# luigiba/OpenKEonSpark

Hardware: AMD Instinct MI355X
Metric: positive triples/sec (training step) (higher is better)
Workload: dtype f32

## Files before the change

### openkeonspark_amd/csrc/abi.hip

```cpp
#include <cstdio>
#include <cstring>
#include <iostream>

#include "engine.hpp"

namespace kge {

Engine &engine() {
    static Engine e;
    return e;
}

void set_error(const std::string &msg) {
    engine().last_error = msg;
    std::fprintf(stderr, "[kge_mi355] error: %s\n", msg.c_str());
}

int fail(int code, const std::string &msg) {
    set_error(msg);
    return code;
}

int hip_check(hipError_t e, const char *what) {
    if (e == hipSuccess) return KGE_OK;
// ... 141 lines not shown
INT getWorkThreads(void) { return engine().work_threads; }
void setBern(INT con) { engine().bern = con; }

void randReset(void) {
    Engine &e = engine();
    e.streams.resize((size_t)e.work_threads);
    for (auto &s : e.streams) s = (uint64_t)(int64_t)e.libc.next();
    e.dev.streams_sync = 0;
}

void importTrainFiles(void) {
    Engine &e = engine();
    std::printf("The toolkit is importing datasets.\n");
    int64_t E = 0, R = 0, nb = 0;
    std::vector<int64_t> h, t, r;
    std::string err = load_openke_dir(e.in_path, E, R, nb, h, t, r);
    if (!err.empty()) {
        std::cout << err << std::endl;
        set_error(err);
        return;
    }
    std::printf("The total of relations is %ld.\n", (long)R);
    std::printf("The total of entities is %ld.\n", (long)E);
    if (nb > 0) std::printf("The total number of new batch triples is: %ld\n", (long)nb);
    std::printf("The total of train triples is %ld.\n", (long)h.size());
    err = build_and_adopt(E, R, nb, (int64_t)h.size(), h.data(), t.data(), r.data());
    if (!err.empty()) { set_error(err); return; }
    std::fflush(stdout);
}

INT getEntityTotal(void) { return engine().index.ent_total; }
INT getRelationTotal(void) { return engine().index.rel_total; }
INT kge_eval_test_total(void); INT kge_eval_valid_total(void); INT kge_eval_triple_total(void);
INT getTripleTotal(void) { return kge_eval_triple_total(); }
INT getTrainTotal(void) { return engine().index.train_uniq; }
INT getTrainTotal_(void) { return engine().index.train_dup; }
INT getBatchTotal(void) { return engine().index.new_batch; }
INT getTestTotal(void) { return kge_eval_test_total(); }
INT getValidTotal(void) { return kge_eval_valid_total(); }

void sampling(INT *batch_h, INT *batch_t, INT *batch_r, REAL *batch_y, INT batchSize, INT negRate, INT negRelRate) {
    Engine &e = engine();
    if (ensure_device_index()) return;
    if (batchSize <= 0 || negRate < 0 || negRelRate < 0) { set_error("sampling: bad sizes"); return; }
    const int64_t total = batchSize * (1 + negRate + negRelRate);
    if (e.dev.stage_i32.reserve(3 * total, "alloc stage")) return;
    if (e.dev.stage_i64.reserve((int64_t)(sizeof(int64_t) * 3 + sizeof(float)) * total, "alloc stage")) return;
    int32_t *s = e.dev.stage_i32;
    if (launch_sampler(s, s + total, s + 2 * total, batchSize, negRate, negRelRate, 0, e.work_threads, batchSize, nullptr, nullptr)) return;
    int64_t *w = reinterpret_cast<int64_t *>(e.dev.stage_i64.ptr());
    if (launch_widen(s, w, batchSize, total, nullptr)) return;
    if (hip_check(hipMemcpy(batch_h, w, sizeof(int64_t) * total, hipMemcpyDeviceToHost), "copy batch_h")) return;
    if (hip_check(hipMemcpy(batch_t, w + total, sizeof(int64_t) * total, hipMemcpyDeviceToHost), "copy batch_t")) return;
    if (hip_check(hipMemcpy(batch_r, w + 2 * total, sizeof(int64_t) * total, hipMemcpyDeviceToHost), "copy batch_r")) return;
    hip_check(hipMemcpy(batch_y, w + 3 * total, sizeof(float) * total, hipMemcpyDeviceToHost), "copy batch_y");
}

size_t kge_last_error(char *buf, size_t n) {
    const std::string &s = engine().last_error;
    if (buf && n) {
        size_t k = s.size() < n - 1 ? s.size() : n - 1;
        std::memcpy(buf, s.data(), k);
        buf[k] = 0;
    }
    return s.size();
}

void kge_clear_error(void) { engine().last_error.clear(); }
int kge_device_available(void) { return device_ok() ? 1 : 0; }
const char *kge_version(void) { return "kge_mi355 0.1 (gfx950)"; }

int kge_set_option(const char *name, INT value) {
    std::string n = name ? name : "";
    if (n == "counts_force_sort") { engine().counts_force_sort = value != 0; return KGE_OK; }
    if (n == "sampler_magic_len") {
        Engine &e = engine();
        if (device_ok()) { (void)flush_attached_sampler(nullptr); (void)hipDeviceSynchronize(); }
        e.sampler_magic_len = value > 0 ? value : 0;
        if (e.index.loaded) build_magic_tables(e.index, e.sampler_magic_len);
        e.dev.tables_uploaded = false;
        return KGE_OK;
    }
    if (n == "counts_sort_tiles") { engine().counts_sort_tiles = value > 0 ? (int)value : 0; return KGE_OK; }
    if (n == "ride_shares") { engine().ride_shares = (int)value; return KGE_OK; }
    if (n == "transr_bf16x3") { engine().transr_bf16x3 = value != 0; return KGE_OK; }
    if (n == "transr_groups") { engine().transr_groups = (int)value; return KGE_OK; }
    if (n == "transr_fuse_vec") { engine().transr_fuse_vec = value != 0; return KGE_OK; }
    if (n == "shared_transr_stages") { engine().shared_transr_stages = value >= 1 && value <= 5 ? (int)value : 5; return KGE_OK; }
    if (n == "counts_fused") { engine().counts_fused = value != 0; return KGE_OK; }
    if (n == "counts_fused_diag") { engine().counts_fused_diag = (int)value; return KGE_OK; }
    if (n == "counts_fused_cap") { engine().counts_fused_cap = value > 0 ? (int)value : 0; return KGE_OK; }
    if (n == "counts_fused_tail") { engine().counts_fused_tail = value != 0; return KGE_OK; }
    if (n == "inv_table_max_bytes") { engine().inv_table_max_bytes = value; return KGE_OK; }
    if (n == "tables_changed") { tables_written(); return KGE_OK; }
    if (n == "counts_krel") { int k = 1; while (k * 2 <= value && k < 64) k *= 2; engine().counts_krel = k; return KGE_OK; }
    if (n == "inv_carry") { engine().inv_carry = value != 0; tables_written(); return KGE_OK; }
    if (n == "emit_rounds") { engine().emit_rounds = value != 0; return KGE_OK; }
    if (n == "emit_pack") { engine().emit_pack = value != 0; return KGE_OK; }
    if (n == "emit_keys_grouped") { engine().emit_keys_grouped = value != 0; return KGE_OK; }
    if (n == "counts_sort_test_group") { engine().counts_sort_test_group = value > 0 ? (int)value : 0; return KGE_OK; }
    if (n == "float_records") { engine().float_records = value != 0; return KGE_OK; }
    if (n == "float_records_min") { engine().float_records_min = value; return KGE_OK; }
    if (n == "index_device_min") { engine().index_device_min = value; return KGE_OK; }
    if (n == "eval_index_device_min") { engine().eval_index_device_min = value; return KGE_OK; }
    if (n == "hub_copies") { engine().hub_copies = value != 0; return KGE_OK; }
    if (n == "pair_counts") { engine().pair_counts = value != 0; return KGE_OK; }
    if (n == "record_emit_event") { engine().record_emit_event = value != 0; return KGE_OK; }
    if (n == "transr_dgrad_records") { engine().transr_dgrad_records = value != 0; return KGE_OK; }
    if (n == "transr_dgrad_records_min") { engine().transr_dgrad_records_min = value; return KGE_OK; }
    if (n == "transr_lean") { engine().transr_lean = value != 0; return KGE_OK; }
    if (n == "pair_counts_min_neg") { engine().pair_counts_min_neg = (int)value; return KGE_OK; }
    if (n == "topk_table_max_bytes") { engine().topk_table_max_bytes = value; return KGE_OK; }
    if (n == "relpred_chunk_bytes") { engine().relpred_chunk_bytes = value; return KGE_OK; }
    if (n == "lp_v1") { engine().lp_v1 = value != 0; return KGE_OK; }
    if (n == "rank_slices") { engine().rank_slices = value > 0 ? (int)value : 0; return KGE_OK; }
    if (n == "rankc_slices") { engine().rankc_slices = value > 0 ? (int)value : 0; return KGE_OK; }
    if (n == "rankc_fused") { engine().rankc_fused = value != 0; return KGE_OK; }
    if (n == "transr_v1") { engine().transr_v1 = (int)value; return KGE_OK; }
    if (n == "time_emit") { engine().time_emit = value > 0 ? (int)value : 0; if (value > 0) { engine().emit_launches = 0; engine().emit_seen = 0; } return KGE_OK; }
    if (n == "time_sampler") { engine().time_sampler = value > 0 ? (int)value : 0; if (value > 0) { engine().samp_launches = 0; engine().samp_seen = 0; } return KGE_OK; }
    if (n == "fb_occ4") { engine().fb_occ4 = value != 0; return KGE_OK; }
    if (n == "persist_ahead") { engine().persist_ahead = value != 0; return KGE_OK; }
    if (n == "persist_touch") { engine().persist_touch = value != 0; return KGE_OK; }
    if (n == "persist_trace") { engine().persist_trace = value != 0; return KGE_OK; }
    if (n == "persist_threads") { engine().persist_threads = value == 1024 ? 1024 : 512; return KGE_OK; }
    if (n == "libc_rand_restart") { engine().libc = LibcRand(); return KGE_OK; }
    return fail(KGE_ERR_BAD_ARG, "kge_set_option: unknown option " + n);
}

int kge_last_kernel_ms(const char *name, float *ms) {
    Engine &e = engine();
    std::string n = name ? name : "";
    if ((n != "transe_emit" && n != "sampler") || !ms) return fail(KGE_ERR_BAD_ARG, "kge_last_kernel_ms: unknown kernel " + n);
    const bool samp = n == "sampler";
    const long long done = samp ? e.samp_launches : e.emit_launches;
    hipEvent_t *ev0 = samp ? e.ev_samp0 : e.ev_emit0, *ev1 = samp ? e.ev_samp1 : e.ev_emit1;
    if (done <= 0) return fail(KGE_ERR_BAD_ARG, "kge_last_kernel_ms: enable option time_emit / time_sampler and run a step first");
    const int slot = (int)((done - 1) % Engine::kEmitRing);
    if (hip_check(hipEventSynchronize(ev1[slot]), "event sync")) return KGE_ERR_NO_DEVICE;
    return hip_check(hipEventElapsedTime(ms, ev0[slot], ev1[slot]), "event elapsed");
}

int kge_kernel_ms_mean(const char *name, float *mean_ms, INT *launches) {
    Engine &e = engine();
    std::string n = name ? name : "";
    if ((n != "transe_emit" && n != "sampler") || !mean_ms) return fail(KGE_ERR_BAD_ARG, "kge_kernel_ms_mean: unknown kernel " + n);
    const bool samp = n == "sampler";
    const long long done = samp ? e.samp_launches : e.emit_launches;
    hipEvent_t *ev0 = samp ? e.ev_samp0 : e.ev_emit0, *ev1 = samp ? e.ev_samp1 : e.ev_emit1;
    const long long have = done < Engine::kEmitRing ? done : (long long)Engine::kEmitRing;
    if (have <= 0) return fail(KGE_ERR_BAD_ARG, "kge_kernel_ms_mean: enable option time_emit / time_sampler and run steps first");
    double sum = 0.0;
    for (long long i = 0; i < have; i++) {
        const int slot = (int)((done - 1 - i) % Engine::kEmitRing);
        float ms = 0.f;
        if (hip_check(hipEventSynchronize(ev1[slot]), "event sync")) return KGE_ERR_NO_DEVICE;
        if (hip_check(hipEventElapsedTime(&ms, ev0[slot], ev1[slot]), "event elapsed")) return KGE_ERR_NO_DEVICE;
        sum += ms;
    }
    *mean_ms = (float)(sum / (double)have);
    if (launches) *launches = have;
    return KGE_OK;
}

int kge_import_train_arrays(INT ent_total, INT rel_total, INT n, const INT *h, const INT *t, const INT *r,
                            INT new_batch_total) {
// ... 339 lines not shown
```

### openkeonspark_amd/csrc/engine.hpp

```cpp
#pragma once
#include <hip/hip_runtime.h>

#include <cstdint>
#include <mutex>
#include <string>
#include <vector>

#include "../../include/kge_mi355.h"
#include "dev_buf.hpp"
#include "kg_index.hpp"

namespace kge {

struct DeviceIndex {
    bool uploaded = false;
    DevBuf<int4> pos, grp;
    DevBuf<int2> ht;
    DevBuf<int32_t> tails_hr, heads_tr, rels_ht;
    DevBuf<float> bern_prob;
    bool tables_uploaded = false;
    DevBuf<LcgAffine> jump_digits;
    DevBuf<uint64_t> ent_magic, rel_magic;
    DevBuf<uint64_t> streams_buf;
    uint64_t *streams = nullptr;
    uint64_t *streams_next = nullptr;
    int streams_sync = 0;
    DevBuf<int32_t> stage_i32;
    DevBuf<char> stage_i64;
    DevBuf<float> loss_partials;
    DevBuf<unsigned> loss_ticket;
    bool typed_uploaded = false;
    DevBuf<int2> typed_len;
    DevBuf<int4> type_bounds;
    DevBuf<int32_t> type_tails, type_heads, typed_pos_hr, typed_pos_tr;
};

struct Engine {
    std::mutex mu;
    std::string in_path = "../data/FB15K/";
    std::string out_path = "../data/FB15K/";
    int64_t work_threads = 1;
    int64_t bern = 0;
    KgIndex index;
    unsigned long long index_generation = 0;
    LibcRand libc;
    std::vector<uint64_t> streams;
    LcgJumpTable jump = make_jump_table();
    std::vector<LcgAffine> jump_digits = make_jump_digit_table(jump);
    int64_t sampler_magic_len = 2048;
    DeviceIndex dev;
    std::string last_error;
    int device_state = 0;
    int record_emit_event = 0;
    hipEvent_t emit_done = nullptr;
    unsigned long long emit_seq = 0, emit_waited = 0;
    int time_emit = 0;
    static constexpr int kEmitRing = 512;
    hipEvent_t ev_emit0[kEmitRing] = {}, ev_emit1[kEmitRing] = {};
    long long emit_launches = 0;
    long long emit_seen = 0;
    int time_sampler = 0;
    hipEvent_t ev_samp0[kEmitRing] = {}, ev_samp1[kEmitRing] = {};
    long long samp_launches = 0, samp_seen = 0;
    DevBuf<float> inv_norm;
    const float *inv_for_ent = nullptr, *inv_for_rel = nullptr;
    int inv_valid = 0;
    int32_t *loss_limbs = nullptr;
    int counts_krel = 4;
    int inv_carry = 1;
    int emit_rounds = 1;
    int emit_pack = 1;
    int emit_keys_grouped = 1;
    int counts_sort_test_group = 0;
    int64_t inv_table_max_bytes = int64_t(256) << 20;
    int float_records = 1;
    int64_t float_records_min = 1 << 16;
    int64_t index_device_min = int64_t(1) << 22;
    int64_t eval_index_device_min = int64_t(1) << 22;
    int transr_dgrad_records = 1;
    int64_t transr_dgrad_records_min = 1 << 15;
    int transr_bf16x3 = 1;
    int transr_groups = 1;
    int transr_fuse_vec = 1;
    int shared_transr_stages = 5;
    int transr_lean = 1;
    int pair_counts = 1;
    int pair_counts_min_neg = 0;
    int hub_copies = 1;
    int64_t topk_table_max_bytes = int64_t(1) << 30;
    int64_t relpred_chunk_bytes = int64_t(256) << 20;
    int lp_v1 = 0;
    int rank_slices = 0;
    int rankc_slices = 0;
    int rankc_fused = 1;
    int transr_v1 = 0;
    int fb_occ4 = 1;
    int persist_ahead = 1;
    int persist_touch = 0;
    int persist_trace = 0;
    int persist_threads = 512;
    int counts_force_sort = 0;
    int counts_sort_tiles = 1;
    int ride_shares = -1;
    int counts_fused = 1;
    int counts_fused_diag = 0;
    int typed_sampling = 0;
    int counts_fused_cap = 0;
    int counts_fused_tail = 1;
};

Engine &engine();
inline void tables_written() { engine().inv_valid = 0; }
struct SamplerArgs;
bool take_attached_sampler(SamplerArgs &a, unsigned &blocks, float share = 1.0f);
int flush_attached_sampler(hipStream_t stream);
int attach_sampler(int32_t *d_h, int32_t *d_t, int32_t *d_r, int64_t B, int64_t neg, int64_t negrel, int64_t thread_lo,
                   int64_t thread_hi, int64_t out_stride, int64_t *n_local_out, hipStream_t stream, int32_t *d_pack = nullptr);
void set_error(const std::string &msg);
int fail(int code, const std::string &msg);
bool device_ok();
int ensure_device_index();
int ensure_typed_index(bool always = false);
int ensure_typed_host_index();
struct TypeListsHost { const std::vector<int32_t> *head_lef, *head_rig, *head_type, *tail_lef, *tail_rig, *tail_type; };
bool eval_type_lists_host(TypeListsHost &v);

constexpr int kMaxLossBlocks = 4096;

struct NegClass { bool same_h, same_t, same_r, fast; };
template <int MODEL>
__host__ __device__ inline NegClass classify_negative(long long h, long long t, long long r, long long nh,
                                                               long long nt, long long nr, int negative_rel) {
    NegClass c;
    c.same_r = nr == r;
    const bool ctx_same = MODEL == KGE_TRANSE ? true : (MODEL == KGE_TRANSR ? (negative_rel == 0 || c.same_r) : c.same_r);
    c.same_h = nh == h && ctx_same;
    c.same_t = nt == t && ctx_same;
    c.fast = ((int)!c.same_h + (int)!c.same_t + (int)!c.same_r) == 1;
    return c;
}



struct FloatRowSpace {
    float *g_ent, *g_rel, *g_auxr, *g_auxe;
    long long E, R;
    long long hub_base, hub_rows;
    long long rows;
    float scale = 1.0f;
};
bool pair_path_active(const kge_model_desc &m, int64_t n_pos, int64_t n_neg);
bool transr_group_layout_active(const kge_model_desc &m, int64_t n_pos, int64_t n_neg);
int transe_relation_copies(const kge_model_desc &m, int64_t n_pos);
int float_records_chunk_len(int64_t M);
int sgd_rows_skipped(int32_t *out);
int float_records_workspace(int64_t M, int D, float *&rec, int32_t *&dst);
int float_records_reduce(int64_t M, int D, const FloatRowSpace &rs, hipStream_t stream, const float *rec_ext = nullptr, int32_t *dst_ext = nullptr,
                         bool deterministic = false);
enum { kRuleAdam = 0, kRuleAdagrad = 1, kRuleRowAdagrad = 2 };
struct RowRule {
    float *m[4], *v[4];
    float lr_t, b1, b2, eps;
    int rule;
};
int float_records_reduce_adam(int64_t M, int D, const FloatRowSpace &rs, const RowRule &ad, hipStream_t stream, const float *rec_ext = nullptr,
                              int32_t *dst_ext = nullptr);
int launch_forward_backward_records(const kge_model_desc &m, const float *const tables[4], const int32_t *d_h, const int32_t *d_t,
                                    const int32_t *d_r, int64_t n_pos, int64_t n_neg, int64_t stride, int64_t denom, int64_t n_pos_total,
                                    float *d_rec, int32_t *d_dst, int64_t rec_offset, int64_t rec_slice, float *d_loss, hipStream_t stream);
int launch_float_records_apply_adam(const kge_model_desc &m, float *const tables[4], const RowRule &ad, const float *d_rec, int32_t *d_dst,
                                    int64_t M_total, int64_t n_pos_total, int64_t n_neg, hipStream_t stream);
int launch_float_records_apply(const kge_model_desc &m, float *const tables[4], const float *d_rec, int32_t *d_dst, int64_t M_total,
                               int64_t n_pos_total, int64_t n_neg, float lr, hipStream_t stream);
void float_record_hubs(const kge_model_desc &m, int64_t n_pos_total, int64_t n_neg, int64_t &hub_base, int64_t &hub_k, int64_t &rows);

bool device_index_build_supported(int64_t E, int64_t R, int64_t n);
std::string build_index_device(KgIndex &ix, DeviceIndex &dev, int64_t E, int64_t R, int64_t new_batch, int64_t n, const int64_t *h,
                               const int64_t *t, const int64_t *r);

int launch_sampler(int32_t *d_h, int32_t *d_t, int32_t *d_r, int64_t B, int64_t neg, int64_t negrel, int64_t thread_lo,
                   int64_t thread_hi, int64_t out_stride, int64_t *n_local, hipStream_t stream, int32_t *d_pack = nullptr);
inline int sampler_kshift(int64_t neg, int64_t negrel) { int k = 0; while ((int64_t(1) << k) < 1 + neg + negrel) k++; return k; }
constexpr int kPackRowBits = 28;
inline bool emit_pack_shape(int64_t ent_total, int64_t rel_total, int64_t neg, int64_t negrel) {
    return engine().emit_pack && sampler_kshift(neg, negrel) <= 6 && neg + negrel >= 1 && ent_total < (int64_t(1) << kPackRowBits) &&
// ... 40 lines not shown
```

### openkeonspark_amd/csrc/transe_counts.hip

```cpp
#include <cstring>
#include <string.h>

#include <rocprim/rocprim.hpp>

#include "engine.hpp"
#include "team.hpp"
#include "team_shape.hpp"
#include "sampler_dev.hpp"
#include "optim_dev.hpp"

namespace kge {

void transe_team_shape(int D, int &L, int &C);
int launch_transe_emit(const kge_model_desc &m, const float *ent, const float *rel, float *resid_ent, float *resid_rel,
                       const int32_t *d_h, const int32_t *d_t, const int32_t *d_r, int64_t n_pos, int64_t n_neg, int64_t stride,
                       int64_t denom, uint32_t *rec, int32_t *dst, int krel, float *d_loss, hipStream_t stream, bool track_deferred,
                       uint8_t *rec2 = nullptr, const int32_t *neg_pack = nullptr, bool keys_grouped = false);
bool transe_emit_groups_keys(int D);

int transe_deferred_groups(int32_t *out);

namespace {

int bits_for_rows(int64_t v) { int b = 1; while ((int64_t(1) << b) <= v) b++; return b; }
// ... 414 lines not shown
        if (threadIdx.x < 64) {
            int v[4], tot = 0;
#pragma unroll
            for (int k = 0; k < 4; k++) { v[k] = span_sum[4 * threadIdx.x + k]; tot += v[k]; }
            int incl = tot;
#pragma unroll
            for (int off = 1; off < 64; off <<= 1) { const int t = __shfl_up(incl, off); if ((int)threadIdx.x >= off) incl += t; }
            int run = incl - tot;
#pragma unroll
            for (int k = 0; k < 4; k++) { span_sum[4 * threadIdx.x + k] = run; run += v[k]; }
        }
        __syncthreads();
        int run = span_sum[threadIdx.x];
        for (int i = lo; i < hi; i++) { const int c = lds_h[i]; lds_h[i] = run; run += c; }
    }
    __syncthreads();
#pragma unroll
    for (int k = 0; k < PC; k++)
        if (start + (int)threadIdx.x + 256 * k < end) {
            const int pos = start + atomicAdd(&lds_h[pr[k].y - row0], 1);
            out_keys[pos] = pr[k].y;
            out_ids[pos] = pr[k].x;
        }
    for (int i = 256 * PC + threadIdx.x; i < n; i += 256) {
        const int2 q = fetch(i);
        const int pos = start + atomicAdd(&lds_h[q.y - row0], 1);
        out_keys[pos] = q.y;
        out_ids[pos] = q.x;
    }
    if constexpr (PLAN) {
        __syncthreads();
        const int cap = plan.cap;
        for (int i = threadIdx.x; i < rpb; i += 256) {
            const int key = row0 + i;
            if (key >= rows) break;
            const int lo = i ? lds_h[i - 1] : 0, c = lds_h[i] - lo;
            plan.row_span[key] = make_int2(start + lo, c);
            const int io = i ^ 1;
            const int co = lds_h[io] - (io ? lds_h[io - 1] : 0);
            if (c > 0 && (c > cap || co > cap)) {
                const int np = (c + cap - 1) / cap;
                const int base = atomicAdd(plan.n_pieces, np);
                for (int q = 0; q < np; q++) plan.pieces[base + q] = make_int4(key, start + lo + q * cap, min(cap, c - q * cap), 0);
            }
            if (plan.expect && !(i & 1)) plan_arrivals(plan, key >> 1, c, co);
        }
    }
}

template <bool PLAN>
__global__ __launch_bounds__(256) void bkt_sort_kernel(const int2 *__restrict__ pairs, const int32_t *__restrict__ bucket_start,
                                                       int rpb, int rows, int32_t *__restrict__ out_keys,
                                                       int32_t *__restrict__ out_ids, int32_t *__restrict__ bucket_total,
                                                       int32_t *__restrict__ cursor, SegPlan plan, SamplerArgs ride) {
    extern __shared__ int lds_h[];
    if ((int)blockIdx.x >= NB) {
        __shared__ float bern_lds[kBernLds];
        sample_block_ride(ride, (long long)blockIdx.x - NB, bern_lds);
        return;
    }
    const int b = blockIdx.x;
    const int row0 = b * rpb;
    if (threadIdx.x == 0) {
        bucket_total[b] = 0; cursor[b] = 0;
        if (b == 0) { bucket_total[NB] = 0; cursor[NB] = 0; }
    }
    if (row0 >= rows) return;
    const int start = bucket_start[b], end = bucket_start[b + 1];
    bucket_rows_sort<PLAN>(row0, start, end, rpb, rows, lds_h, out_keys, out_ids, plan, [&](int i) { return pairs[start + i]; });
}


template <bool PLAN>
static void launch_bkt_sort(int2 *pairs, int rpb, int rows, int32_t *totals, int32_t *cursor, const SegPlan &plan, hipStream_t stream) {
    SamplerArgs ride = {};
    const unsigned n_ride = take_ride(ride, 2);
    hipLaunchKernelGGL(bkt_sort_kernel<PLAN>, dim3(NB + n_ride), dim3(256), sizeof(int) * (size_t)rpb, stream, pairs, g_c.bucket_start, rpb, rows,
                       g_c.dst_sorted, g_c.ids_sorted, totals, cursor, plan, ride);
}

constexpr int kSortTile = 2048;
constexpr int kSortMaxTiles = 2048;
constexpr int kOffStride = NB + 1;

struct KeyMap {
    unsigned S, magic, shift;
    int n_pos;
};
static KeyMap key_map_for(int S, int64_t n_pos) {
    KeyMap k;
    k.S = (unsigned)S; k.n_pos = (int)n_pos;
    unsigned sh = 0;
    while ((2u << sh) <= (unsigned)S) sh++;
    if ((1u << sh) == (unsigned)S) { k.magic = 0x80000000u; k.shift = sh - 1; }
    else {
        k.magic = (unsigned)(((uint64_t(1) << (32 + sh)) + (unsigned)S - 1) / (unsigned)S); k.shift = sh;
    }
    return k;
}
__device__ __forceinline__ int key_id_of(unsigned S, unsigned magic, unsigned shift, int n_pos, int p) {
    const unsigned b = __umulhi((unsigned)p, magic) >> shift;
    return (int)(((unsigned)p - b * S) * (unsigned)n_pos + b);
}

template <int T, bool GROUPED = false>
__global__ __launch_bounds__(256) void bkt_tile_kernel(const int32_t *__restrict__ dst, int M, int rpb, int2 *__restrict__ tile_pairs,
                                                       int32_t *__restrict__ tile_off, int32_t *__restrict__ plan_counter, SamplerArgs ride,
                                                       int n_tiles, unsigned km_S, unsigned km_magic, unsigned km_shift, int km_n_pos) {
    if ((int)blockIdx.x >= n_tiles) {
        __shared__ float bern_lds[kBernLds];
        sample_block_ride(ride, (long long)blockIdx.x - n_tiles, bern_lds);
        return;
    }
    constexpr int K = T / 256;
    __shared__ int hist[NB];
    __shared__ int wave_total[4];
    __shared__ int2 stage[T];
    if (plan_counter && blockIdx.x == 0 && threadIdx.x == 0) plan_counter[0] = 0;
    const int base = blockIdx.x * T;
    int d[K], code[K];
#pragma unroll
    for (int k = 0; k < K; k++) {
        const int m = base + threadIdx.x + 256 * k;
        d[k] = m < M ? dst[m] : -1;
    }
    for (int i = threadIdx.x; i < NB; i += 256) hist[i] = 0;
    __syncthreads();
#pragma unroll
    for (int k = 0; k < K; k++) {
        const unsigned bk = (unsigned)d[k] / (unsigned)rpb;
        code[k] = bk < (unsigned)NB ? (int)(bk << 16) | atomicAdd(&hist[bk], 1) : -1;
    }
    __syncthreads();
    {
        const int v0 = hist[2 * threadIdx.x], v1 = hist[2 * threadIdx.x + 1], run = v0 + v1;
        const int lane = threadIdx.x & 63, wave = threadIdx.x >> 6;
        int incl = run;
#pragma unroll
        for (int off = 1; off < 64; off <<= 1) { const int t = __shfl_up(incl, off); if (lane >= off) incl += t; }
        if (lane == 63) wave_total[wave] = incl;
        __syncthreads();
        int excl = incl - run;
        for (int w = 0; w < wave; w++) excl += wave_total[w];
        hist[2 * threadIdx.x] = excl; hist[2 * threadIdx.x + 1] = excl + v0;
        int32_t *off = tile_off + (size_t)blockIdx.x * kOffStride;
        off[2 * threadIdx.x] = excl; off[2 * threadIdx.x + 1] = excl + v0;
        if (threadIdx.x == 255) off[NB] = excl + run;
    }
    __syncthreads();
    const int live = wave_total[0] + wave_total[1] + wave_total[2] + wave_total[3];
#pragma unroll
    for (int k = 0; k < K; k++)
        if (code[k] >= 0) {
            const int p = base + (int)threadIdx.x + 256 * k;
            stage[hist[code[k] >> 16] + (code[k] & 0xFFFF)] = make_int2(GROUPED ? key_id_of(km_S, km_magic, km_shift, km_n_pos, p) : p, d[k]);
        }
    __syncthreads();
    for (int i = threadIdx.x; i < live; i += 256) tile_pairs[base + i] = stage[i];
}

template <bool PLAN, int T>
__global__ __launch_bounds__(256) void bkt_merge_kernel(const int2 *__restrict__ tile_pairs, const int32_t *__restrict__ tile_off, int n_tiles,
                                                        int32_t *__restrict__ bucket_start, int M, int rpb, int rows,
                                                        int32_t *__restrict__ out_keys, int32_t *__restrict__ out_ids, SegPlan plan,
                                                        SamplerArgs ride) {
    extern __shared__ int lds_h[];
    if ((int)blockIdx.x >= NB) {
        __shared__ float bern_lds[kBernLds];
        sample_block_ride(ride, (long long)blockIdx.x - NB, bern_lds);
        return;
    }
    __shared__ int seg_pre[kSortMaxTiles + 1];
    __shared__ int seg_src[kSortMaxTiles];
    __shared__ int wave_len[4], wave_below[4];
    const int b = blockIdx.x;
    constexpr int PER = kSortMaxTiles / 256;
    const int per = (n_tiles + 255) / 256;
    const int t_lo = min((int)threadIdx.x * per, n_tiles), t_hi = min(t_lo + per, n_tiles);
    int a[PER], e[PER];
#pragma unroll
    for (int j = 0; j < PER; j++) {
        const int32_t *off = tile_off + (size_t)min(t_lo + j, max(n_tiles - 1, 0)) * kOffStride + b;
        const bool mine = t_lo + j < t_hi;
        a[j] = mine ? off[0] : 0;
        e[j] = mine ? off[1] : 0;
    }
    int len = 0, below = 0;
#pragma unroll
    for (int j = 0; j < PER; j++)
        if (t_lo + j < t_hi) {
            seg_src[t_lo + j] = (t_lo + j) * T + a[j];
            seg_pre[t_lo + j] = len;
            len += e[j] - a[j];
            below += a[j];
        }
    const int lane = threadIdx.x & 63, wave = threadIdx.x >> 6;
    int incl = len;
#pragma unroll
    for (int off = 1; off < 64; off <<= 1) { const int t = __shfl_up(incl, off); if (lane >= off) incl += t; }
#pragma unroll
    for (int off = 32; off > 0; off >>= 1) below += __shfl_xor(below, off);
    if (lane == 63) { wave_len[wave] = incl; wave_below[wave] = below; }
    __syncthreads();
    int excl = incl - len;
    for (int w = 0; w < wave; w++) excl += wave_len[w];
    for (int t = t_lo; t < t_hi; t++) seg_pre[t] += excl;
    const int start = wave_below[0] + wave_below[1] + wave_below[2] + wave_below[3];
    const int end = start + wave_len[0] + wave_len[1] + wave_len[2] + wave_len[3];
    if (threadIdx.x == 0) {
        seg_pre[n_tiles] = end - start;
        bucket_start[b] = start;
        if (b == NB - 1) { bucket_start[NB] = end; bucket_start[NB + 1] = M; }
    }
    __syncthreads();
    const int row0 = b * rpb;
    if (row0 >= rows) return;
    bucket_rows_sort<PLAN>(row0, start, end, rpb, rows, lds_h, out_keys, out_ids, plan, [&](int i) {
        int lo = 0, hi = n_tiles;
        while (hi - lo > 1) { const int mid = (lo + hi) >> 1; if (seg_pre[mid] <= i) lo = mid; else hi = mid; }
        return tile_pairs[seg_src[lo] + (i - seg_pre[lo])];
    });
}

template <int T>
static void launch_tile_sort(const int32_t *dst, int n_tiles, int M, int rows, int rpb, const SegPlan *plan, hipStream_t stream,
                             const KeyMap *km) {
    int2 *pairs = reinterpret_cast<int2 *>(g_c.pairs.ptr());
    SamplerArgs ride = {};
    unsigned n_ride = take_ride(ride, 1, true);
    if (n_tiles + n_ride > 0) {
        if (km)
            hipLaunchKernelGGL((bkt_tile_kernel<T, true>), dim3((unsigned)n_tiles + n_ride), dim3(256), 0, stream, dst, M, rpb, pairs,
                               g_c.tile_off.ptr(), plan ? plan->n_pieces : nullptr, ride, n_tiles, km->S, km->magic, km->shift, km->n_pos);
        else
            hipLaunchKernelGGL((bkt_tile_kernel<T, false>), dim3((unsigned)n_tiles + n_ride), dim3(256), 0, stream, dst, M, rpb, pairs,
                               g_c.tile_off.ptr(), plan ? plan->n_pieces : nullptr, ride, n_tiles, 0u, 0u, 0u, 0);
    }
    ride = SamplerArgs();
    n_ride = take_ride(ride, 2, true);
    if (plan)
        hipLaunchKernelGGL((bkt_merge_kernel<true, T>), dim3(NB + n_ride), dim3(256), sizeof(int) * (size_t)rpb, stream, pairs, g_c.tile_off.ptr(),
                           n_tiles, g_c.bucket_start.ptr(), M, rpb, rows, g_c.dst_sorted.ptr(), g_c.ids_sorted.ptr(), *plan, ride);
    else
        hipLaunchKernelGGL((bkt_merge_kernel<false, T>), dim3(NB + n_ride), dim3(256), sizeof(int) * (size_t)rpb, stream, pairs, g_c.tile_off.ptr(),
                           n_tiles, g_c.bucket_start.ptr(), M, rpb, rows, g_c.dst_sorted.ptr(), g_c.ids_sorted.ptr(), SegPlan(), ride);
}

__global__ void run_flags_kernel(const int32_t *__restrict__ keys, const int32_t *__restrict__ n_valid_p, int M, int32_t *__restrict__ flags) {
    const int n = n_valid_p[0];
    for (int i = blockIdx.x * blockDim.x + threadIdx.x; i < M; i += gridDim.x * blockDim.x)
        flags[i] = (i < n && (i == 0 || keys[i] != keys[i - 1])) ? 1 : 0;
}

__global__ void unique_rows_kernel(const int32_t *__restrict__ keys, const int32_t *__restrict__ n_valid_p, int32_t *__restrict__ uidx1,
                                   int32_t *__restrict__ rows_out, int32_t *__restrict__ n_rows_out, int32_t *__restrict__ S, int D,
                                   int32_t *__restrict__ bflag) {
    const int n = n_valid_p[0];
    for (int i = blockIdx.x * blockDim.x + threadIdx.x; i < n; i += gridDim.x * blockDim.x) {
        const int u = uidx1[i] - 1;
        uidx1[i] = u;
        if (i == 0 || keys[i] != keys[i - 1]) rows_out[u] = keys[i];
        if (i == n - 1) n_rows_out[0] = u + 1;
        if (bflag && ((i % CHUNK) == 0 || (i % CHUNK) == CHUNK - 1 || i == n - 1)) bflag[u] = 1;
    }
    if (n == 0 && blockIdx.x == 0 && threadIdx.x == 0) n_rows_out[0] = 0;
}

__global__ __launch_bounds__(256) void zero_boundary_rows_kernel(const int32_t *__restrict__ uidx, const int32_t *__restrict__ n_valid_p,
                                                                 int32_t *__restrict__ S, int D) {
    const int n = n_valid_p[0];
    const int lane = threadIdx.x & 63;
    const long long n_chunks = ((long long)n + CHUNK - 1) / CHUNK;
    for (long long c = (long long)blockIdx.x * 4 + (threadIdx.x >> 6); c < n_chunks; c += (long long)gridDim.x * 4) {
        const long long first = c * CHUNK, last = min(first + CHUNK, (long long)n) - 1;
        const int u0 = uidx[first], u1 = uidx[last];
        for (int e = lane; e < D; e += 64) {
            S[(long long)u0 * D + e] = 0;
            S[(long long)u1 * D + e] = 0;
        }
    }
}



__device__ __forceinline__ float *float_row_ptr(const FloatRowSpace &rs, long long row, int D) {
    if (row < rs.E) return rs.g_ent + row * D;
    if (row < rs.hub_base) return rs.g_auxe + (row - rs.E) * D;
    const long long q = (row - rs.hub_base) % rs.hub_rows;
    return q < rs.R ? rs.g_rel + q * D : rs.g_auxr + (q - rs.R) * D;
}

template <int L, int C>
__device__ __forceinline__ void flush_run_f32(const FloatRowSpace &rs, int D, int lane, long long row, const float (&acc)[C], bool atomic) {
    float *p = float_row_ptr(rs, row, D);
    atomic = atomic || row >= rs.hub_base;
#pragma unroll
    for (int c = 0; c < C; c++) {
        const int e = lane + L * c;
        if (e < D) {
            const float v = mul_rn(rs.scale, acc[c]);
            if (atomic) __builtin_amdgcn_global_atomic_fadd_f32((__attribute__((address_space(1))) float *)(p + e), v);
            else p[e] += v;
        }
    }
}

template <int L, int C>
__global__ __launch_bounds__(256) void segsum_f32_kernel(const float *__restrict__ rec, const int32_t *__restrict__ keys,
                                                         const int32_t *__restrict__ ids, const int32_t *__restrict__ n_valid_p,
                                                         FloatRowSpace rs, int D, int chunk_len) {
    constexpr int TEAMS = 256 / L;
    constexpr int U = C <= 4 ? 8 : 4;
    const int lane = threadIdx.x % L;
    const int n_valid = n_valid_p[0];
    const long long chunk = (long long)blockIdx.x * TEAMS + threadIdx.x / L;
    const long long start = chunk * chunk_len;
    if (start >= n_valid) return;
    const int n = (int)min((long long)chunk_len, n_valid - start);
    float acc[C];
#pragma unroll
    for (int c = 0; c < C; c++) acc[c] = 0.f;
    int cur = keys[start];
    bool first_run = true;
    constexpr int J = CHUNK / L;
    int kl[J], idl[J];
#pragma unroll
    for (int j = 0; j < J; j++) {
// ... 364 lines not shown
        q.row = row; q.rel = rel;
        if (row != req_row) {
            req_x = *reinterpret_cast<const float4 *>(pr.ent + (long long)row * D + lane4);
            if constexpr (MODEL == KGE_TRANSD) req_xa = *reinterpret_cast<const float4 *>(pr.auxe + (long long)row * D + lane4);
            req_row = row;
        }
        q.x = req_x;
        if constexpr (MODEL == KGE_TRANSD) q.xa = req_xa;
        q.cw = *reinterpret_cast<const float4 *>(pr.ctx + (long long)rel * D + lane4);
        q.signs = 0;
#pragma unroll
        for (int u = 0; u < W; u++) {
            const long long id = __builtin_amdgcn_readlane(idl, min(lo + u, hi - 1));
            q.w[u] = load_record(id, q.signs, u);
            if (u == 0) q.ai = pr.aux[id];
        }
    };
    auto next_run = [&](int &lo, int &hi) {
        lo = __ffsll((long long)starts) - 1;
        starts &= starts - 1;
        hi = starts ? __ffsll((long long)starts) - 1 : n;
    };
    Pair cur;
    { int lo, hi; next_run(lo, hi); request(cur, lo, hi); }
    for (;;) {
        const bool more = starts != 0;
        Pair nxt;
        if (more) { int lo, hi; next_run(lo, hi); request(nxt, lo, hi); }
        int acc[4];
#pragma unroll
        for (int j = 0; j < 4; j++) acc[j] = elem(cur.w[0], cur.signs & 1, j);
        if (cur.hi - cur.lo > 1) {
#pragma unroll
            for (int u = 1; u < W; u++) {
                if (cur.lo + u < cur.hi) {
#pragma unroll
                    for (int j = 0; j < 4; j++) acc[j] += elem(cur.w[u], (cur.signs >> u) & 1, j);
                }
            }
        }
        for (int i = cur.lo + W; i < cur.hi; i++) {
            const long long id = __builtin_amdgcn_readlane(idl, i);
            int kind = 0;
            const uint32_t w = load_record(id, kind, 0);
#pragma unroll
            for (int j = 0; j < 4; j++) acc[j] += elem(w, kind & 1, j);
        }
        if (cur.row != cur_row) {
            if (cur_row >= 0) { flush_row(first_row); first_row = false; }
            cur_row = cur.row;
        }
        const float4 z = make_float4(0.f, 0.f, 0.f, 0.f);
        const float4 x = valid ? cur.x : z, cw = valid ? cur.cw : z;
        float4 xa = z, xp;
        const float a = cur.ai.x;
        const bool uc = cur.ai.y > 0.f;
        const float inv = fabsf(cur.ai.y);
        if constexpr (MODEL == KGE_TRANSH) {
            xp = make_float4(x.x - a * cw.x, x.y - a * cw.y, x.z - a * cw.z, x.w - a * cw.w);
        } else {
            xa = valid ? cur.xa : z;
            xp = make_float4(x.x + a * cw.x, x.y + a * cw.y, x.z + a * cw.z, x.w + a * cw.w);
        }
        const float4 S = make_float4((float)acc[0], (float)acc[1], (float)acc[2], (float)acc[3]);
        const float dp = team_sum<L>(dot4(xp, S));
        const float al = uc ? inv * pr.unit * dp : 0.f;
        const float cg = inv * pr.unit, cx = -inv * inv * al;
        const float4 gxp = make_float4(cg * S.x + cx * xp.x, cg * S.y + cx * xp.y, cg * S.z + cx * xp.z, cg * S.w + cx * xp.w);
        const float d = team_sum<L>(dot4(gxp, cw));
        if constexpr (MODEL == KGE_TRANSH) {
            racc.x += gxp.x - d * cw.x; racc.y += gxp.y - d * cw.y; racc.z += gxp.z - d * cw.z; racc.w += gxp.w - d * cw.w;
        } else {
            racc.x += gxp.x + d * xa.x; racc.y += gxp.y + d * xa.y; racc.z += gxp.z + d * xa.z; racc.w += gxp.w + d * xa.w;
            racc2.x += d * x.x; racc2.y += d * x.y; racc2.z += d * x.z; racc2.w += d * x.w;
        }
        if (!more) break;
        cur = nxt;
    }
    flush_row(true);
}


static int sort_tile_size() { const int opt = engine().counts_sort_tiles; return opt == 1024 || opt == 4096 ? opt : kSortTile; }
bool sort_takes_tiles(int64_t M) { return engine().counts_sort_tiles != 0 && (M + sort_tile_size() - 1) / sort_tile_size() <= kSortMaxTiles; }
int bucket_sort_records(const int32_t *dst, int64_t M, int rows, int rpb, const SegPlan *plan, hipStream_t stream, const int32_t *&n_live,
                        const KeyMap *km = nullptr) {
    int rc;
    bool grew;
    if ((rc = g_c.bucket_start.reserve(NB + 2, "counts bucket_start"))) return rc;
    n_live = g_c.bucket_start + NB;
    const int T = sort_tile_size();
    const int64_t n_tiles_new = (M + T - 1) / T;
    if (sort_takes_tiles(M)) {
        if ((rc = g_c.tile_off.reserve((n_tiles_new + 1) * kOffStride, "counts tile offsets"))) return rc;
        if (T == 1024) launch_tile_sort<1024>(dst, (int)n_tiles_new, (int)M, rows, rpb, plan, stream, km);
        else if (T == 4096) launch_tile_sort<4096>(dst, (int)n_tiles_new, (int)M, rows, rpb, plan, stream, km);
        else launch_tile_sort<kSortTile>(dst, (int)n_tiles_new, (int)M, rows, rpb, plan, stream, km);
        return KGE_OK;
    }
    if (km) return fail(KGE_ERR_UNSUPPORTED, "record sort: group-major keys need the two-launch form");
    if ((rc = g_c.tile_hist.reserve(2 * (NB + 2), "counts bucket totals/cursors", &grew))) return rc;
    if (grew && (rc = hip_check(hipMemset(g_c.tile_hist, 0, sizeof(int32_t) * 2 * (NB + 2)), "zero bucket totals"))) { g_c.tile_hist.free(); return rc; }
    const int n_tiles = (int)((M + BTILE - 1) / BTILE);
    int32_t *totals = g_c.tile_hist, *cursor = g_c.tile_hist + (NB + 2);
    int2 *pairs = reinterpret_cast<int2 *>(g_c.pairs.ptr());
    launch_bkt_hist(dst, n_tiles, (int)M, rpb, totals, plan ? plan->n_pieces : nullptr, stream);
    launch_bkt_scatter(dst, n_tiles, (int)M, rpb, totals, cursor, pairs, stream);
    if (plan) launch_bkt_sort<true>(pairs, rpb, rows, totals, cursor, *plan, stream);
    else launch_bkt_sort<false>(pairs, rpb, rows, totals, cursor, SegPlan(), stream);
    return KGE_OK;
}

int radix_sort_records(int32_t *dst, int64_t M, int rows, bool blank, const char *what, hipStream_t stream, const int32_t *&n_live) {
    int blocks = (int)((M + 255) / 256);
    if (blocks > 4096) blocks = 4096;
    if (blank) hipLaunchKernelGGL(blank_keys_kernel, dim3(blocks), dim3(256), 0, stream, dst, (long long)M, rows);
    else hipLaunchKernelGGL(fix_keys_kernel, dim3(blocks), dim3(256), 0, stream, dst, (long long)M, rows);
    size_t tmp = (size_t)g_c.sort_tmp.cap();
    int rc = hip_check(rocprim::radix_sort_pairs(g_c.sort_tmp.ptr(), tmp, dst, g_c.dst_sorted.ptr(), g_c.ids.ptr(), g_c.ids_sorted.ptr(), (size_t)M, 0,
                                                 bits_for_rows(rows), stream), what);
    if (rc) return rc;
    hipLaunchKernelGGL(count_valid_kernel, dim3(1), dim3(64), 0, stream, g_c.dst_sorted, (int)M, rows, g_c.n_valid);
    n_live = g_c.n_valid;
    return KGE_OK;
}

int ensure_hub_sums(size_t need, hipStream_t stream) {
    bool grew;
    int rc = g_c.hub_sums.reserve((int64_t)need, "hub copy sums", &grew);
    if (!rc && grew && (rc = hip_check(hipMemsetAsync(g_c.hub_sums, 0, sizeof(float) * need, stream), "zero hub copy sums"))) g_c.hub_sums.free();
    return rc;
}

template <int L, int C, int V, int RULE>
void launch_segsum_rule(int64_t M, const float *rec, const FloatRowSpace &rs, const RowRule &ad, int D, int K, hipStream_t stream) {
    long long nb = (M + (256 / L) - 1) / (256 / L);
    if (nb > 16384) nb = 16384;
    hipLaunchKernelGGL((segsum_adam_runs_kernel<L, C, V, RULE>), dim3((unsigned)nb), dim3(256), 0, stream, rec, g_c.dst_sorted,
                       g_c.ids_sorted, g_c.n_valid, rs, ad, D, g_c.hub_sums, g_c.hub_marks);
    if (K > 0) {
        long long nf = (rs.hub_rows + (256 / L) - 1) / (256 / L);
        if (nf > 16384) nf = 16384;
        hipLaunchKernelGGL((hub_fold_adam_kernel<L, C, V, RULE>), dim3((unsigned)nf), dim3(256), 0, stream, g_c.hub_sums, g_c.hub_marks,
                           rs, ad, D, K);
    }
}
template <int L, int C, int V>
void launch_segsum_adam(int64_t M, const float *rec, const FloatRowSpace &rs, const RowRule &ad, int D, int K, hipStream_t stream) {
    if (ad.rule == kRuleAdagrad) launch_segsum_rule<L, C, V, kRuleAdagrad>(M, rec, rs, ad, D, K, stream);
    else if (ad.rule == kRuleRowAdagrad) launch_segsum_rule<L, C, V, kRuleRowAdagrad>(M, rec, rs, ad, D, K, stream);
    else launch_segsum_rule<L, C, V, kRuleAdam>(M, rec, rs, ad, D, K, stream);
}

}

int float_records_chunk_len(int64_t M) { return M >= (int64_t(1) << 20) ? 64 : (M >= (int64_t(1) << 18) ? 32 : 16); }

int transe_relation_copies(const kge_model_desc &m, int64_t n_pos) {
    int krel = 1;
    if (n_pos >= 4096 && m.rel_total > 0 && engine().counts_krel > 1) {
        krel = engine().counts_krel;
        while (krel > 1 && (int64_t)krel * m.rel_total > 2 * (m.ent_total + m.rel_total)) krel >>= 1;
    }
    return krel;
}

int float_records_workspace(int64_t M, int D, float *&rec, int32_t *&dst) {
    int rc = ensure_counts_work(M, (size_t)D);
    if (rc) return rc;
    rec = reinterpret_cast<float *>(g_c.rec.ptr());
    dst = g_c.dst;
    return KGE_OK;
}

int float_records_reduce(int64_t M, int D, const FloatRowSpace &rs, hipStream_t stream, const float *rec_ext, int32_t *dst_ext, bool deterministic) {
    int rc;
    const bool ext = rec_ext && dst_ext;
    if (ext && (rc = ensure_counts_work(M, 0))) return rc;
    const float *rec = ext ? rec_ext : reinterpret_cast<const float *>(g_c.rec.ptr());
    int32_t *dst = ext ? dst_ext : g_c.dst.ptr();
// ... 1022 lines not shown
```

Baseline: 181.1 million.

## Store per-tile bucket offsets blocked and packed, remap merge buckets across XCDs

The tile-sort offset table moves from a tile-major layout with one int per bucket boundary to a bucket-block-major layout. Each cell packs start and length into one 32-bit word, so merge blocks read contiguous runs of G buckets across tiles instead of strided rows. The merge kernel also permutes blockIdx so consecutive XCD-interleaved blocks handle contiguous bucket ranges, which should improve L2 locality on offset reads. Packing limits tile size to under 65536, and the new path is on by default behind a new option.

```diff
diff --git a/openkeonspark_amd/csrc/abi.hip b/openkeonspark_amd/csrc/abi.hip
--- a/openkeonspark_amd/csrc/abi.hip
+++ b/openkeonspark_amd/csrc/abi.hip
@@ -247,6 +247,7 @@
         return KGE_OK;
     }
     if (n == "counts_sort_tiles") { engine().counts_sort_tiles = value > 0 ? (int)value : 0; return KGE_OK; }
+    if (n == "counts_sort_blocked") { engine().counts_sort_blocked = value > 0 ? (int)value : 0; return KGE_OK; }
     if (n == "ride_shares") { engine().ride_shares = (int)value; return KGE_OK; }
     if (n == "transr_bf16x3") { engine().transr_bf16x3 = value != 0; return KGE_OK; }
     if (n == "transr_groups") { engine().transr_groups = (int)value; return KGE_OK; }
diff --git a/openkeonspark_amd/csrc/engine.hpp b/openkeonspark_amd/csrc/engine.hpp
--- a/openkeonspark_amd/csrc/engine.hpp
+++ b/openkeonspark_amd/csrc/engine.hpp
@@ -101,6 +101,7 @@
     int persist_threads = 512;
     int counts_force_sort = 0;
     int counts_sort_tiles = 1;
+    int counts_sort_blocked = 1;
     int ride_shares = -1;
     int counts_fused = 1;
     int counts_fused_diag = 0;
diff --git a/openkeonspark_amd/csrc/transe_counts.hip b/openkeonspark_amd/csrc/transe_counts.hip
--- a/openkeonspark_amd/csrc/transe_counts.hip
+++ b/openkeonspark_amd/csrc/transe_counts.hip
@@ -520,6 +520,7 @@
 constexpr int kSortTile = 2048;
 constexpr int kSortMaxTiles = 2048;
 constexpr int kOffStride = NB + 1;
+constexpr int kSortBlock = 8;
 
 struct KeyMap {
     unsigned S, magic, shift;
@@ -541,7 +542,7 @@
     return (int)(((unsigned)p - b * S) * (unsigned)n_pos + b);
 }
 
-template <int T, bool GROUPED = false>
+template <int T, bool GROUPED = false, int G = 0>
 __global__ __launch_bounds__(256) void bkt_tile_kernel(const int32_t *__restrict__ dst, int M, int rpb, int2 *__restrict__ tile_pairs,
                                                        int32_t *__restrict__ tile_off, int32_t *__restrict__ plan_counter, SamplerArgs ride,
                                                        int n_tiles, unsigned km_S, unsigned km_magic, unsigned km_shift, int km_n_pos) {
@@ -550,6 +551,8 @@
         sample_block_ride(ride, (long long)blockIdx.x - n_tiles, bern_lds);
         return;
     }
+    static_assert(T < 65536, "a cell's start and length share one 32-bit word");
+    static_assert(G == 0 || (G % 2 == 0 && NB % G == 0), "a thread's two buckets lie in one block");
     constexpr int K = T / 256;
     __shared__ int hist[NB];
     __shared__ int wave_total[4];
@@ -581,9 +584,15 @@
         int excl = incl - run;
         for (int w = 0; w < wave; w++) excl += wave_total[w];
         hist[2 * threadIdx.x] = excl; hist[2 * threadIdx.x + 1] = excl + v0;
-        int32_t *off = tile_off + (size_t)blockIdx.x * kOffStride;
-        off[2 * threadIdx.x] = excl; off[2 * threadIdx.x + 1] = excl + v0;
-        if (threadIdx.x == 255) off[NB] = excl + run;
+        if constexpr (G > 0) {
+            const int b0 = 2 * threadIdx.x;
+            int32_t *pk = tile_off + ((size_t)(b0 / G) * n_tiles + blockIdx.x) * G + b0 % G;
+            *reinterpret_cast<int2 *>(pk) = make_int2(excl | (v0 << 16), (excl + v0) | (v1 << 16));
+        } else {
+            int32_t *off = tile_off + (size_t)blockIdx.x * kOffStride;
+            off[2 * threadIdx.x] = excl; off[2 * threadIdx.x + 1] = excl + v0;
+            if (threadIdx.x == 255) off[NB] = excl + run;
+        }
     }
     __syncthreads();
     const int live = wave_total[0] + wave_total[1] + wave_total[2] + wave_total[3];
@@ -597,7 +606,7 @@
     for (int i = threadIdx.x; i < live; i += 256) tile_pairs[base + i] = stage[i];
 }
 
-template <bool PLAN, int T>
+template <bool PLAN, int T, int G = 0>
 __global__ __launch_bounds__(256) void bkt_merge_kernel(const int2 *__restrict__ tile_pairs, const int32_t *__restrict__ tile_off, int n_tiles,
                                                         int32_t *__restrict__ bucket_start, int M, int rpb, int rows,
                                                         int32_t *__restrict__ out_keys, int32_t *__restrict__ out_ids, SegPlan plan,
@@ -611,17 +620,25 @@
     __shared__ int seg_pre[kSortMaxTiles + 1];
     __shared__ int seg_src[kSortMaxTiles];
     __shared__ int wave_len[4], wave_below[4];
-    const int b = blockIdx.x;
+    static_assert(NB % 8 == 0 && (G == 0 || NB % G == 0), "the XCD runs and the offset blocks tile the buckets");
+    const int b = G > 0 ? ((int)blockIdx.x % 8) * (NB / 8) + (int)blockIdx.x / 8 : (int)blockIdx.x;
     constexpr int PER = kSortMaxTiles / 256;
     const int per = (n_tiles + 255) / 256;
     const int t_lo = min((int)threadIdx.x * per, n_tiles), t_hi = min(t_lo + per, n_tiles);
     int a[PER], e[PER];
 #pragma unroll
     for (int j = 0; j < PER; j++) {
-        const int32_t *off = tile_off + (size_t)min(t_lo + j, max(n_tiles - 1, 0)) * kOffStride + b;
+        const int tc = min(t_lo + j, max(n_tiles - 1, 0));
         const bool mine = t_lo + j < t_hi;
-        a[j] = mine ? off[0] : 0;
-        e[j] = mine ? off[1] : 0;
+        if constexpr (G > 0) {
+            const unsigned w = mine ? (unsigned)tile_off[((size_t)(b / G) * n_tiles + tc) * G + b % G] : 0u;
+            a[j] = (int)(w & 0xFFFFu);
+            e[j] = a[j] + (int)(w >> 16);
+        } else {
+            const int32_t *off = tile_off + (size_t)tc * kOffStride + b;
+            a[j] = mine ? off[0] : 0;
+            e[j] = mine ? off[1] : 0;
+        }
     }
     int len = 0, below = 0;
 #pragma unroll
@@ -660,7 +677,7 @@
     });
 }
 
-template <int T>
+template <int T, int G>
 static void launch_tile_sort(const int32_t *dst, int n_tiles, int M, int rows, int rpb, const SegPlan *plan, hipStream_t stream,
                              const KeyMap *km) {
     int2 *pairs = reinterpret_cast<int2 *>(g_c.pairs.ptr());
@@ -668,19 +685,19 @@
     unsigned n_ride = take_ride(ride, 1, true);
     if (n_tiles + n_ride > 0) {
         if (km)
-            hipLaunchKernelGGL((bkt_tile_kernel<T, true>), dim3((unsigned)n_tiles + n_ride), dim3(256), 0, stream, dst, M, rpb, pairs,
+            hipLaunchKernelGGL((bkt_tile_kernel<T, true, G>), dim3((unsigned)n_tiles + n_ride), dim3(256), 0, stream, dst, M, rpb, pairs,
                                g_c.tile_off.ptr(), plan ? plan->n_pieces : nullptr, ride, n_tiles, km->S, km->magic, km->shift, km->n_pos);
         else
-            hipLaunchKernelGGL((bkt_tile_kernel<T, false>), dim3((unsigned)n_tiles + n_ride), dim3(256), 0, stream, dst, M, rpb, pairs,
+            hipLaunchKernelGGL((bkt_tile_kernel<T, false, G>), dim3((unsigned)n_tiles + n_ride), dim3(256), 0, stream, dst, M, rpb, pairs,
                                g_c.tile_off.ptr(), plan ? plan->n_pieces : nullptr, ride, n_tiles, 0u, 0u, 0u, 0);
     }
     ride = SamplerArgs();
     n_ride = take_ride(ride, 2, true);
     if (plan)
-        hipLaunchKernelGGL((bkt_merge_kernel<true, T>), dim3(NB + n_ride), dim3(256), sizeof(int) * (size_t)rpb, stream, pairs, g_c.tile_off.ptr(),
+        hipLaunchKernelGGL((bkt_merge_kernel<true, T, G>), dim3(NB + n_ride), dim3(256), sizeof(int) * (size_t)rpb, stream, pairs, g_c.tile_off.ptr(),
                            n_tiles, g_c.bucket_start.ptr(), M, rpb, rows, g_c.dst_sorted.ptr(), g_c.ids_sorted.ptr(), *plan, ride);
     else
-        hipLaunchKernelGGL((bkt_merge_kernel<false, T>), dim3(NB + n_ride), dim3(256), sizeof(int) * (size_t)rpb, stream, pairs, g_c.tile_off.ptr(),
+        hipLaunchKernelGGL((bkt_merge_kernel<false, T, G>), dim3(NB + n_ride), dim3(256), sizeof(int) * (size_t)rpb, stream, pairs, g_c.tile_off.ptr(),
                            n_tiles, g_c.bucket_start.ptr(), M, rpb, rows, g_c.dst_sorted.ptr(), g_c.ids_sorted.ptr(), SegPlan(), ride);
 }
 
@@ -1211,6 +1228,7 @@
 
 
 static int sort_tile_size() { const int opt = engine().counts_sort_tiles; return opt == 1024 || opt == 4096 ? opt : kSortTile; }
+static int sort_block_size() { const int opt = engine().counts_sort_blocked; return opt == 4 || opt == 16 ? opt : opt ? kSortBlock : 0; }
 bool sort_takes_tiles(int64_t M) { return engine().counts_sort_tiles != 0 && (M + sort_tile_size() - 1) / sort_tile_size() <= kSortMaxTiles; }
 int bucket_sort_records(const int32_t *dst, int64_t M, int rows, int rpb, const SegPlan *plan, hipStream_t stream, const int32_t *&n_live,
                         const KeyMap *km = nullptr) {
@@ -1221,10 +1239,19 @@
     const int T = sort_tile_size();
     const int64_t n_tiles_new = (M + T - 1) / T;
     if (sort_takes_tiles(M)) {
-        if ((rc = g_c.tile_off.reserve((n_tiles_new + 1) * kOffStride, "counts tile offsets"))) return rc;
-        if (T == 1024) launch_tile_sort<1024>(dst, (int)n_tiles_new, (int)M, rows, rpb, plan, stream, km);
-        else if (T == 4096) launch_tile_sort<4096>(dst, (int)n_tiles_new, (int)M, rows, rpb, plan, stream, km);
-        else launch_tile_sort<kSortTile>(dst, (int)n_tiles_new, (int)M, rows, rpb, plan, stream, km);
+        const int G = sort_block_size();
+        if ((rc = g_c.tile_off.reserve(G ? (n_tiles_new + 1) * NB : (n_tiles_new + 1) * kOffStride, "counts tile offsets"))) return rc;
+        const int n_tiles = (int)n_tiles_new;
+        if (T == 1024) {
+            if (G) launch_tile_sort<1024, kSortBlock>(dst, n_tiles, (int)M, rows, rpb, plan, stream, km);
+            else launch_tile_sort<1024, 0>(dst, n_tiles, (int)M, rows, rpb, plan, stream, km);
+        } else if (T == 4096) {
+            if (G) launch_tile_sort<4096, kSortBlock>(dst, n_tiles, (int)M, rows, rpb, plan, stream, km);
+            else launch_tile_sort<4096, 0>(dst, n_tiles, (int)M, rows, rpb, plan, stream, km);
+        } else if (G == 4) launch_tile_sort<kSortTile, 4>(dst, n_tiles, (int)M, rows, rpb, plan, stream, km);
+        else if (G == 16) launch_tile_sort<kSortTile, 16>(dst, n_tiles, (int)M, rows, rpb, plan, stream, km);
+        else if (G) launch_tile_sort<kSortTile, kSortBlock>(dst, n_tiles, (int)M, rows, rpb, plan, stream, km);
+        else launch_tile_sort<kSortTile, 0>(dst, n_tiles, (int)M, rows, rpb, plan, stream, km);
         return KGE_OK;
     }
     if (km) return fail(KGE_ERR_UNSUPPORTED, "record sort: group-major keys need the two-launch form");
```

Result: no change. 185.7 million, median of 6 (+2.5%).
